# InhwanBae/EigenTrajectory

Hardware: AMD Instinct MI355X
Metric: trajectories/sec fit+project+reconstruct+kmeans (higher is better)
Workload: dtype f32

## Files before the change

### eigentrajectory_amd/csrc/et_fit.hip

```cpp
#include "et_common.h"

namespace et {

constexpr int kFitThreads = 256;

template <int TO, int TP>
struct GramLayout {
    static constexpr int DO = 2 * TO, DP = 2 * TP, D = DO + DP;
    static constexpr int kPairs = 10;
    static constexpr int kSums = kPairs * 64;
    static constexpr int kPartial = kSums + 1;
};
__host__ __device__ constexpr int gram4_block(int s, int q) { return s == 0 ? q : 4 + (s == 1 ? q : (s == 2 ? (q < 2 ? 4 + q : q - 2) : 2 + q)); }
__host__ __device__ constexpr int gram4_pair(int qa, int qb) { return qa * 4 - qa * (qa - 1) / 2 + (qb - qa); }

constexpr int kWaveGramThreads = 256;

__device__ __forceinline__ float4 ld_rows(const float4 *p) { return *p; }

typedef float f32x2_t __attribute__((ext_vector_type(2)));
struct NormPk {
    f32x2_t o, cc, sn, sc;
    __device__ __forceinline__ explicit NormPk(const RowNorm &p)
        : o{p.ox, p.oy}, cc{p.c, p.c}, sn{p.s, -p.s}, sc{p.mv ? p.sca : 1.0f, p.mv ? p.sca : 1.0f} {}
    __device__ __forceinline__ f32x2_t point(f32x2_t xy) const {
        const f32x2_t t = xy - o;
        return (t * cc + __builtin_shufflevector(t, t, 1, 0) * sn) * sc;
    }
    __device__ __forceinline__ float4 quad(float x0, float y0, float x1, float y1) const {
        const f32x2_t a = point((f32x2_t){x0, y0}), b = point((f32x2_t){x1, y1});
        return make_float4(a.x, a.y, b.x, b.y);
    }
};

template <int TO, int TP>
__global__ __launch_bounds__(kWaveGramThreads) void gram_wave_kernel(
    const float *__restrict__ obs, const float *__restrict__ pred, int64_t N, int mode, float static_dist, int which,
    double *__restrict__ partials) {
    using L = GramLayout<TO, TP>;
    static_assert(TO == 8 && TP == 12, "the MFMA tiling below is laid out for 16 + 24 features");
    constexpr int DO = L::DO, DP = L::DP;
    constexpr int QO = DO / 4, QP = DP / 4;
    constexpr int kWaves = kWaveGramThreads / 64;
    constexpr int PR = QO + QP + 1;
    static_assert(PR % 2 == 1, "the row pitch must be odd in float4 units");
    constexpr int kSliceF4 = 64 * PR;
    constexpr int kRedDoubles = kWaves * L::kSums;
    constexpr int kLdsDoubles = (2 * kWaves * kSliceF4 > kRedDoubles ? 2 * kWaves * kSliceF4 : kRedDoubles) + 2;
    __shared__ __attribute__((aligned(16))) double sMem[kLdsDoubles];
    double *sRed = sMem;
    int *sCountPtr = reinterpret_cast<int *>(sMem + kLdsDoubles - 2);

    const int tid = threadIdx.x;
    const int lane = tid & 63, wave = tid >> 6;
    const int kslot = lane >> 4;
    float4 *sRow = reinterpret_cast<float4 *>(sMem) + wave * kSliceF4;
    double acc[L::kPairs];
#pragma unroll
    for (int t = 0; t < L::kPairs; ++t) acc[t] = 0.0;
    const int opi = lane & 3, opslot = (lane >> 2) & 3;
    const int rowA = kslot == 0 ? 0 : (kslot == 1 ? 3 : (kslot == 2 ? 6 : 1)), rowB = rowA ^ 4;
    int offA[4], offB[4];
#pragma unroll
    for (int q = 0; q < 4; ++q) {
        offA[q] = rowA * (4 * PR) + 4 * gram4_block(opslot, q) + opi;
        offB[q] = rowB * (4 * PR) + 4 * gram4_block(opslot, q) + opi;
    }
    int my_count = 0;
    const int64_t n_tiles = ceil_div(N, (int64_t)64);
    const int64_t first = (int64_t)blockIdx.x * kWaves + wave, stride = (int64_t)gridDim.x * kWaves;
    float4 ro[QO], rp[QP];
    auto fetch = [&](int64_t tile) {
        const int64_t n0 = tile * 64;
        const int rows = (int)min((int64_t)64, N - n0);
        const float4 *go = reinterpret_cast<const float4 *>(obs + n0 * DO);
        const float4 *gp = reinterpret_cast<const float4 *>(pred + n0 * DP);
        if (rows == 64) {
#pragma unroll
            for (int j = 0; j < QO; ++j) ro[j] = ld_rows(go + lane + j * 64);
#pragma unroll
            for (int j = 0; j < QP; ++j) rp[j] = ld_rows(gp + lane + j * 64);
        } else {
#pragma unroll
            for (int j = 0; j < QO; ++j) ro[j] = lane + j * 64 < rows * QO ? ld_rows(go + lane + j * 64) : make_float4(0.f, 0.f, 0.f, 0.f);
#pragma unroll
            for (int j = 0; j < QP; ++j) rp[j] = lane + j * 64 < rows * QP ? ld_rows(gp + lane + j * 64) : make_float4(0.f, 0.f, 0.f, 0.f);
        }
    };
    auto wave_sync = [&]() {
        __builtin_amdgcn_fence(__ATOMIC_RELEASE, "wavefront");
        __builtin_amdgcn_wave_barrier();
        __builtin_amdgcn_fence(__ATOMIC_ACQUIRE, "wavefront");
    };
    if (first < n_tiles) fetch(first);
    for (int64_t tile = first; tile < n_tiles; tile += stride) {
        const int rows = (int)min((int64_t)64, N - tile * 64);
        wave_sync();
#pragma unroll
        for (int j = 0; j < QO; ++j) {
            const int q = lane + j * 64;
            sRow[(q / QO) * PR + (q % QO)] = ro[j];
        }
#pragma unroll
        for (int j = 0; j < QP; ++j) {
            const int q = lane + j * 64;
            sRow[(q / QP) * PR + QO + (q % QP)] = rp[j];
        }
        if (tile + stride < n_tiles) fetch(tile + stride);
        wave_sync();
        float4 *orow = sRow + lane * PR, *prow = orow + QO;
        bool use = false;
        if (lane < rows) {
            float xo[DO];
#pragma unroll
            for (int j = 0; j < QO; ++j) {
                const float4 v = orow[j];
                xo[4 * j] = v.x;
                xo[4 * j + 1] = v.y;
                xo[4 * j + 2] = v.z;
                xo[4 * j + 3] = v.w;
            }
            const float ox = xo[DO - 2], oy = xo[DO - 1];
            const RowNorm p = row_norm(ox, oy, ox - xo[DO - 6], oy - xo[DO - 5], mode, static_dist);
            use = p.mv == which;
            if (use) {
                const NormPk np(p);
#pragma unroll
                for (int j = 0; j < QO; ++j) orow[j] = np.quad(xo[4 * j], xo[4 * j + 1], xo[4 * j + 2], xo[4 * j + 3]);
#pragma unroll
                for (int q = 0; q < QP; ++q) {
                    const float4 v = prow[q];
                    prow[q] = np.quad(v.x, v.y, v.z, v.w);
                }
                ++my_count;
            }
        }
        if (!use) {
            const float4 z = make_float4(0.f, 0.f, 0.f, 0.f);
#pragma unroll
            for (int j = 0; j < QO; ++j) orow[j] = z;
#pragma unroll
            for (int q = 0; q < QP; ++q) prow[q] = z;
        }
        wave_sync();
        const float *fb = reinterpret_cast<const float *>(sRow);
#pragma unroll
        for (int g = 0; g < 16; ++g) {
            const int wo = (g >> 1) * (8 * 4 * PR);
            double v[4];
#pragma unroll
            for (int q = 0; q < 4; ++q) v[q] = (double)fb[((g & 1) ? offB[q] : offA[q]) + wo];
#pragma unroll
            for (int qa = 0; qa < 4; ++qa)
#pragma unroll
                for (int qb = qa; qb < 4; ++qb)
                    acc[gram4_pair(qa, qb)] = __builtin_amdgcn_mfma_f64_4x4x4f64(v[qa], v[qb], acc[gram4_pair(qa, qb)], 0, 0, 0);
        }
    }

    __syncthreads();
    if (tid == 0) *sCountPtr = 0;
    __syncthreads();
#pragma unroll
    for (int t = 0; t < L::kPairs; ++t) sRed[wave * L::kSums + t * 64 + lane] = acc[t];
    if (my_count) atomicAdd(sCountPtr, my_count);
    __syncthreads();
    double *dst = partials + (size_t)blockIdx.x * L::kPartial;
    for (int i = tid; i < L::kSums; i += kWaveGramThreads) {
        double sum = 0.0;
        for (int w = 0; w < kWaves; ++w) sum += sRed[w * L::kSums + i];
        dst[i] = sum;
    }
    if (tid == 0) dst[L::kSums] = (double)*sCountPtr;
}

__device__ __forceinline__ double gram4_slot_entry(const double *S, int s, int pa, int ia, int pb, int jb) {
    if (pa > pb || (pa == pb && ia > jb)) {
        int t = pa;
        pa = pb;
        pb = t;
        t = ia;
        ia = jb;
        jb = t;
    }
    return S[gram4_pair(pa, pb) * 64 + jb + 4 * s + 16 * ia];
}
__device__ __forceinline__ double gram_obs_entry(const double *S, int i, int j) { return gram4_slot_entry(S, 0, i >> 2, i & 3, j >> 2, j & 3); }
__device__ __forceinline__ double gram_pred_entry(const double *S, int i, int j) {
    if (i > j) {
        const int t = i;
        i = j;
        j = t;
    }
    const int ba = i >> 2, bb = j >> 2;
    for (int s = 1; s < 4; ++s) {
        int pa = -1, pb = -1;
        for (int q = 0; q < 4; ++q) {
            if (gram4_block(s, q) == 4 + ba) pa = q;
            if (gram4_block(s, q) == 4 + bb) pb = q;
        }
        if (pa >= 0 && pb >= 0) return gram4_slot_entry(S, s, pa, i & 3, pb, j & 3);
    }
    return 0.0;
}

__global__ __launch_bounds__(64) void gram_reduce_kernel(const double *__restrict__ partials, int n_partials, int stride,
                                                         double *__restrict__ sums) {
    const int e = blockIdx.x;
    double s = 0.0;
    for (int b = threadIdx.x; b < n_partials; b += 64) s += partials[(size_t)b * stride + e];
    for (int o = 32; o > 0; o >>= 1) s += __shfl_xor(s, o);
    if (threadIdx.x == 0) sums[e] = s;
}

template <int TO, int TP>
__global__ __launch_bounds__(kFitThreads) void gram_finish_kernel(const double *__restrict__ sSum,
                                                                  double *__restrict__ G_obs,
                                                                  double *__restrict__ G_pred,
                                                                  int64_t *__restrict__ count) {
    using L = GramLayout<TO, TP>;
    constexpr int DO = L::DO, DP = L::DP;
    for (int e = threadIdx.x; e < DO * DO; e += kFitThreads) G_obs[e] = gram_obs_entry(sSum, e / DO, e % DO);
    for (int e = threadIdx.x; e < DP * DP; e += kFitThreads) G_pred[e] = gram_pred_entry(sSum, e / DP, e % DP);
    if (threadIdx.x == 0) *count = (int64_t)sSum[L::kSums];
}

__global__ __launch_bounds__(kFitThreads) void gram_generic_kernel(
    const float *__restrict__ obs, const float *__restrict__ pred, int64_t N, int T_obs, int T_pred, int mode,
    float static_dist, int which, double *__restrict__ partials) {
    constexpr int kSlab = 32;
    const int DO = 2 * T_obs, DP = 2 * T_pred, D = DO + DP;
    extern __shared__ __attribute__((aligned(16))) double sF[];
    int &sCnt = *reinterpret_cast<int *>(sF + kSlab * D);
    const int tid = threadIdx.x;
    const int n_entries = DO * DO + DP * DP;
    double *dst = partials + (size_t)blockIdx.x * (n_entries + 1);
    for (int e = tid; e < n_entries + 1; e += kFitThreads) dst[e] = 0.0;
    if (tid == 0) sCnt = 0;
    const int64_t n_slabs = ceil_div(N, (int64_t)kSlab);
    for (int64_t slab = blockIdx.x; slab < n_slabs; slab += gridDim.x) {
        const int64_t n0 = slab * kSlab;
        const int rows = (int)min((int64_t)kSlab, N - n0);
        __syncthreads();
        if (tid < kSlab) {
            double *f = sF + tid * D;
            bool use = false;
            if (tid < rows) {
                const float *row = obs + (n0 + tid) * DO;
                const float ox = row[DO - 2], oy = row[DO - 1];
                const RowNorm p = row_norm(ox, oy, ox - row[DO - 6], oy - row[DO - 5], mode, static_dist);
                use = p.mv == which;
                if (use) {
                    for (int t = 0; t < T_obs; ++t) {
                        float a, b;
                        normalize_point(p, row[2 * t], row[2 * t + 1], a, b);
                        f[2 * t] = (double)a;
                        f[2 * t + 1] = (double)b;
                    }
                    const float *prow = pred + (n0 + tid) * DP;
                    for (int t = 0; t < T_pred; ++t) {
                        float a, b;
                        normalize_point(p, prow[2 * t], prow[2 * t + 1], a, b);
                        f[DO + 2 * t] = (double)a;
                        f[DO + 2 * t + 1] = (double)b;
                    }
                    atomicAdd(&sCnt, 1);
                }
            }
            if (!use)
                for (int e = 0; e < D; ++e) f[e] = 0.0;
        }
        __syncthreads();
        for (int e = tid; e < n_entries; e += kFitThreads) {
            int i, j;
            if (e < DO * DO) {
                i = e / DO;
                j = e % DO;
            } else {
                const int r = e - DO * DO;
                i = DO + r / DP;
                j = DO + r % DP;
            }
            double s = dst[e];
            for (int r = 0; r < kSlab; ++r) s = fma(sF[r * D + i], sF[r * D + j], s);
            dst[e] = s;
        }
    }
    __syncthreads();
    if (tid == 0) dst[n_entries] = (double)sCnt;
}

__global__ __launch_bounds__(kFitThreads) void gram_generic_finish_kernel(const double *__restrict__ sums, int DO, int DP,
                                                                          double *__restrict__ G_obs,
                                                                          double *__restrict__ G_pred,
                                                                          int64_t *__restrict__ count) {
    const int n_entries = DO * DO + DP * DP;
    for (int e = threadIdx.x; e < n_entries + 1; e += kFitThreads) {
        const double s = sums[e];
        if (e < DO * DO) G_obs[e] = s;
        else if (e < n_entries) G_pred[e - DO * DO] = s;
        else *count = (int64_t)s;
    }
}

constexpr int kJacobiMaxSweeps = 30;
constexpr double kJacobiStop = 1e-10;
constexpr int kEighThreads = 1024;

__device__ __forceinline__ void sqrt_rsqrt(double x, double &root, double &rroot) {
    const double y = __builtin_amdgcn_rsq(x);
    double g = x * y, h = 0.5 * y;
    double r = fma(-h, g, 0.5);
    g = fma(g, r, g);
    h = fma(h, r, h);
    r = fma(-h, g, 0.5);
    g = fma(g, r, g);
    h = fma(h, r, h);
    root = g;
    rroot = h + h;
}

__device__ __forceinline__ void jacobi_schedule(int m, int r, int i, int &p, int &q) {
    int a, b;
    if (i == 0) {
        a = m - 1;
        b = r;
    } else {
        a = r + i;
        a = a >= m - 1 ? a - (m - 1) : a;
        b = r + (m - 1) - i;
        b = b >= m - 1 ? b - (m - 1) : b;
    }
    p = a < b ? a : b;
    q = a < b ? b : a;
}

struct JacobiPair {
    int a, b;
    bool fixed;
    __device__ __forceinline__ void init(int m, int i) {
        fixed = i == 0;
        a = i;
        b = i == 0 ? 0 : m - 1 - i;
    }
    __device__ __forceinline__ void get(int m, int &p, int &q) const {
        const int ae = fixed ? m - 1 : a;
        p = ae < b ? ae : b;
        q = ae < b ? b : ae;
    }
    __device__ __forceinline__ void step(int m) {
        const unsigned a1 = (unsigned)a + 1u, b1 = (unsigned)b + 1u, w = (unsigned)(m - 1);
        a = (int)min(a1, a1 - w);
        b = (int)min(b1, b1 - w);
    }
};

template <class GLoad>
__device__ __forceinline__ void eigh_topk_body(GLoad gload, int n, int k, float *__restrict__ U, float *__restrict__ sigma,
                                               double *sm) {
    const int lane = threadIdx.x;
    const int m = (n + 1) & ~1, half = m / 2;
    double *Abuf = sm;
    double *V = sm + 2 * m * m;
    double *sC = V + m * m;
    double *sS = sC + 64;
    unsigned long long *sMax = reinterpret_cast<unsigned long long *>(sS + 64);
    int *sAct = reinterpret_cast<int *>(sMax + 4);
    int *sUsed = sAct + 64;
    uint2 *sTab = reinterpret_cast<uint2 *>(sUsed + 64);
    for (int i = lane; i < m * m; i += kEighThreads) {
        const int r = i / m, c = i - r * m;
        Abuf[i] = (r < n && c < n) ? gload(r, c) : 0.0;
        V[i] = (r == c && r < n) ? 1.0 : 0.0;
    }
    if (lane < 4) sMax[lane] = 0ull;
    const int nItems = 3 * half;
    for (int idx = lane; idx < (m - 1) * nItems; idx += kEighThreads) {
        const int r = idx / nItems, it = idx - r * nItems, e = it / half, Lt = it - e * half;
        int p, q;
        jacobi_schedule(m, r + 1 == m - 1 ? 0 : r + 1, Lt, p, q);
        int i1 = 0, p1 = 0, q1 = 0, i2 = 0, p2 = 0, q2 = 0;
        for (int i = 0; i < half; ++i) {
            int pi, qi;
            jacobi_schedule(m, r, i, pi, qi);
            if (p == pi || p == qi) { i1 = i; p1 = pi; q1 = qi; }
            if (q == pi || q == qi) { i2 = i; p2 = pi; q2 = qi; }
        }
        const int iR = e == 2 ? i2 : i1, pR = e == 2 ? p2 : p1, qR = e == 2 ? q2 : q1;
        const int iC = e == 1 ? i1 : i2, pC = e == 1 ? p1 : p2, qC = e == 1 ? q1 : q2;
        const unsigned row2 = (e == 2 ? q : p) == qR, col2 = (e == 1 ? p : q) == qC, zero = e == 0 && i1 == i2;
        sTab[idx] = make_uint2((unsigned)(pR * m + pC) | (unsigned)(pR * m + qC) << 12 | (unsigned)iR << 24,
                               (unsigned)(qR * m + pC) | (unsigned)(qR * m + qC) << 12 | (unsigned)iC << 24 | row2 << 29 |
                                   col2 << 30 | zero << 31);
    }
    __syncthreads();
    static_assert(kEighThreads == 1024, "the V items are dealt to wavefronts 4 ... 14 of sixteen");
    constexpr int kVPerSlot = 9 * 64;
    constexpr int kSlots = (32 * 64 + kVPerSlot - 1) / kVPerSlot;
    constexpr int kBlkSlots = (32 * 32 + kEighThreads - 1) / kEighThreads;
    constexpr int kChkSlots = (64 * 64 + kEighThreads - 1) / kEighThreads;
    constexpr int kParBase = kEighThreads - 64;
    int slot_i[kSlots], slot_row[kSlots], blk_1[kBlkSlots], blk_2[kBlkSlots], chk[kChkSlots];
#pragma unroll
    for (int t = 0; t < kSlots; ++t) {
        const int w = lane >> 6;
        const int e = (w >= 4 && (w & 3) != 3) ? ((w - 4) - ((w - 4) >> 2)) * 64 + (lane & 63) + t * kVPerSlot : -1;
        const bool ok = e >= 0 && e < half * n;
        slot_i[t] = ok ? e / n : -1;
        slot_row[t] = ok ? (e % n) * m : 0;
    }
#pragma unroll
    for (int t = 0; t < kBlkSlots; ++t) {
        const int b = lane + t * kEighThreads;
        blk_1[t] = b < half * half ? b / half : -1;
        blk_2[t] = b < half * half ? b % half : 0;
    }
    JacobiPair b1[kBlkSlots], b2[kBlkSlots];
#pragma unroll
    for (int t = 0; t < kBlkSlots; ++t) {
        b1[t].init(m, blk_1[t] < 0 ? 0 : blk_1[t]);
        b2[t].init(m, blk_2[t]);
    }
    const int pl = lane - kParBase;
    const bool split = 4 * half <= 64;
    const bool is_par = pl >= 0 && (split ? (pl & 3) == 0 && (pl >> 2) < half : pl < half);
    const int L = is_par ? (split ? pl >> 2 : pl) : 0;
    const int item0 = pl < 0 ? 0 : (split ? ((pl & 3) < 3 && (pl >> 2) < half ? (pl & 3) * half + (pl >> 2) : 0) : (pl < half ? pl : 0));
    JacobiPair par;
    par.init(m, L);
#pragma unroll
    for (int t = 0; t < kChkSlots; ++t) {
        const int e = lane + t * kEighThreads;
        const int i = e / n, j = e - i * n;
        chk[t] = (e < n * n && j >= i) ? (i * m + j) | (i == j ? 1 << 20 : 0) : -1;
    }
    auto rotation = [&](double apq, double app, double aqq, int buf) {
        const double alpha = aqq - app, beta = 2.0 * apq;
        double h, rh;
        sqrt_rsqrt(alpha * alpha + beta * beta, h, rh);
        const double D = fabs(alpha) + h;
        double g, rg;
        sqrt_rsqrt(D * D + beta * beta, g, rg);
        const double sgn = (alpha == 0.0 || ((alpha > 0.0) == (beta > 0.0))) ? 1.0 : -1.0;
        const bool act = apq != 0.0;
        sC[buf * 32 + L] = act ? D * rg : 1.0;
        sS[buf * 32 + L] = act ? sgn * fabs(beta) * rg : 0.0;
        sAct[buf * 32 + L] = act ? 1 : 0;
    };
    int cur = 0, pb = 0;
    if (pl >= 0) __builtin_amdgcn_s_setprio(3);
    if (is_par) {
        int p, q;
        par.get(m, p, q);
        rotation(Abuf[__mul24(p, m) + q], Abuf[__mul24(p, m) + p], Abuf[__mul24(q, m) + q], 0);
    }
    uint2 ent[3] = {sTab[item0], sTab[split ? item0 : half + item0], sTab[split ? item0 : 2 * half + item0]};
    for (int sweep = 0; sweep < kJacobiMaxSweeps; ++sweep) {
        const double *Ac = Abuf + cur * m * m;
        unsigned long long *mx = sMax + 2 * (sweep & 1);
#pragma unroll
        for (int t = 0; t < kChkSlots; ++t) {
            if (chk[t] < 0) continue;
            const unsigned long long bits = static_cast<unsigned long long>(__double_as_longlong(fabs(Ac[chk[t] & 0xfffff])));
            atomicMax(mx + (chk[t] >> 20), bits);
        }
        if (lane < 2) sMax[2 * ((sweep + 1) & 1) + lane] = 0ull;
        __syncthreads();
        const double off = __longlong_as_double(static_cast<long long>(mx[0])), diag = __longlong_as_double(static_cast<long long>(mx[1]));
        if (off <= kJacobiStop * diag) break;
        for (int r = 0; r < m - 1; ++r) {
            const double *Ar = Abuf + cur * m * m;
            double *Aw = Abuf + (cur ^ 1) * m * m;
            const double *pC = sC + pb * 32, *pS = sS + pb * 32;
            const int *pAct = sAct + pb * 32;
            if (pl >= 0) {
                auto entry = [&](uint2 t) -> double {
                    const double x_pp = Ar[t.x & 0xfffu], x_pq = Ar[(t.x >> 12) & 0xfffu];
                    const double x_qp = Ar[t.y & 0xfffu], x_qq = Ar[(t.y >> 12) & 0xfffu];
                    const int iR = (int)((t.x >> 24) & 31u), iC = (int)((t.y >> 24) & 31u);
                    const double cR = pC[iR], sR = pS[iR], cC = pC[iC], sC_ = pS[iC];
                    const int actR = pAct[iR];
                    const bool row2 = (t.y >> 29) & 1u, col2 = (t.y >> 30) & 1u;
                    const double alR = row2 ? sR : cR, beR = row2 ? cR : -sR;
                    const double alC = col2 ? sC_ : cC, beC = col2 ? cC : -sC_;
                    const double v = alC * (alR * x_pp + beR * x_qp) + beC * (alR * x_pq + beR * x_qq);
                    return ((t.y >> 31) & (unsigned)actR) ? 0.0 : v;
                };
                double apq, app, aqq;
                if (split) {
                    const double v = entry(ent[0]);
                    const int lo = __double2loint(v), hi = __double2hiint(v);
                    apq = v;
                    app = __hiloint2double(__builtin_amdgcn_mov_dpp(hi, 0x55, 0xf, 0xf, false), __builtin_amdgcn_mov_dpp(lo, 0x55, 0xf, 0xf, false));
                    aqq = __hiloint2double(__builtin_amdgcn_mov_dpp(hi, 0xaa, 0xf, 0xf, false), __builtin_amdgcn_mov_dpp(lo, 0xaa, 0xf, 0xf, false));
                } else {
                    apq = entry(ent[0]);
                    app = entry(ent[1]);
                    aqq = entry(ent[2]);
                }
                const int rn = r + 1 == m - 1 ? 0 : r + 1;
                ent[0] = sTab[rn * nItems + item0];
                if (!split) {
                    ent[1] = sTab[rn * nItems + half + item0];
                    ent[2] = sTab[rn * nItems + 2 * half + item0];
                }
                if (is_par) rotation(apq, app, aqq, pb ^ 1);
            }
#pragma unroll
            for (int t = 0; t < kBlkSlots; ++t) {
                const int i1 = blk_1[t], i2 = blk_2[t];
                if (i1 < 0) continue;
                int p1, q1, p2, q2;
                b1[t].get(m, p1, q1);
                b2[t].get(m, p2, q2);
                const int rp = __mul24(p1, m), rq = __mul24(q1, m);
                const int diag_act = pAct[i1] & (i1 == i2 ? 1 : 0);
                const double c1 = pC[i1], s1 = pS[i1], c2 = pC[i2], s2 = pS[i2];
                const double x_pp = Ar[rp + p2], x_pq = Ar[rp + q2], x_qp = Ar[rq + p2], x_qq = Ar[rq + q2];
                const double t_pp = c1 * x_pp - s1 * x_qp, t_qp = s1 * x_pp + c1 * x_qp;
                const double t_pq = c1 * x_pq - s1 * x_qq, t_qq = s1 * x_pq + c1 * x_qq;
                const double r_pp = c2 * t_pp - s2 * t_pq, r_qp = c2 * t_qp - s2 * t_qq;
                double r_pq = s2 * t_pp + c2 * t_pq, r_qp2 = r_qp;
                const double r_qq = s2 * t_qp + c2 * t_qq;
                if (diag_act) {
                    r_pq = 0.0;
                    r_qp2 = 0.0;
                }
                Aw[rp + p2] = r_pp;
                Aw[rp + q2] = r_pq;
                Aw[rq + p2] = r_qp2;
                Aw[rq + q2] = r_qq;
            }
#pragma unroll
            for (int t = 0; t < kSlots; ++t) {
                const int i = slot_i[t];
                if (i < 0) continue;
                int p, q;
                jacobi_schedule(m, r, i, p, q);
                const double c = pC[i], sn = pS[i];
                double *row = V + slot_row[t];
                const double vjp = row[p], vjq = row[q];
                row[p] = c * vjp - sn * vjq;
                row[q] = sn * vjp + c * vjq;
            }
#pragma unroll
            for (int t = 0; t < kBlkSlots; ++t) {
                b1[t].step(m);
                b2[t].step(m);
            }
            __syncthreads();
            cur ^= 1;
            pb ^= 1;
        }
    }
    double *A = Abuf + cur * m * m;
    __syncthreads();
    if (lane < n) {
        const double di = A[lane * m + lane];
        int rank = 0;
        for (int i = 0; i < n; ++i) {
            const double dj = A[i * m + i];
            rank += (dj > di || (dj == di && i < lane)) ? 1 : 0;
        }
        sUsed[lane] = rank;
    }
    __syncthreads();
    for (int e = lane; e < n * k; e += kEighThreads) {
        const int col = e / k, j = e - col * k;
        if (sUsed[col] != j) continue;
        int im = 0;
        for (int i = 1; i < n; ++i)
            if (fabs(V[i * m + col]) > fabs(V[im * m + col])) im = i;
        const double sgn = V[im * m + col] < 0.0 ? -1.0 : 1.0;
        const double lam = A[col * m + col];
        sigma[j] = (float)sqrt(lam > 0.0 ? lam : 0.0);
        for (int i = 0; i < n; ++i) U[i * k + j] = (float)(sgn * V[i * m + col]);
    }
}

__global__ __launch_bounds__(kEighThreads) void eigh_topk_kernel(const double *__restrict__ G, int n, int k,
                                                                  float *__restrict__ U, float *__restrict__ sigma) {
    extern __shared__ __attribute__((aligned(16))) double eigh_smem[];
    eigh_topk_body([=](int r, int c) { return G[r * n + c]; }, n, k, U, sigma, eigh_smem);
}

struct EighBatch {
    const double *G[ET_EIGH_MAX_BATCH];
    float *U[ET_EIGH_MAX_BATCH];
    float *sigma[ET_EIGH_MAX_BATCH];
    int n[ET_EIGH_MAX_BATCH];
    int k[ET_EIGH_MAX_BATCH];
};

__global__ __launch_bounds__(kEighThreads) void eigh_topk_batch_kernel(const EighBatch b) {
    extern __shared__ __attribute__((aligned(16))) double eigh_smem[];
    const int i = blockIdx.x;
    const double *G = b.G[i];
    const int n = b.n[i];
    eigh_topk_body([=](int r, int c) { return G[r * n + c]; }, n, b.k[i], b.U[i], b.sigma[i], eigh_smem);
}

template <int TO, int TP>
__global__ __launch_bounds__(kEighThreads) void fit_finish_eigh_kernel(const double *__restrict__ sums, int k,
                                                                       double *__restrict__ G_obs, double *__restrict__ G_pred,
                                                                       int64_t *__restrict__ count, float *__restrict__ U_obs,
                                                                       float *__restrict__ U_pred, float *__restrict__ sigma_obs,
                                                                       float *__restrict__ sigma_pred) {
    using L = GramLayout<TO, TP>;
    constexpr int DO = L::DO, DP = L::DP;
    extern __shared__ __attribute__((aligned(16))) double eigh_smem[];
    double *sT = eigh_smem;
    const bool is_pred = blockIdx.x == 1;
    for (int e = threadIdx.x; e < L::kSums; e += kEighThreads) sT[e] = sums[e];
    if (!is_pred && count && threadIdx.x == 0) *count = (int64_t)sums[L::kSums];
    __syncthreads();
    if (!is_pred) {
        if (G_obs)
            for (int e = threadIdx.x; e < DO * DO; e += kEighThreads) G_obs[e] = gram_obs_entry(sT, e / DO, e % DO);
        eigh_topk_body([=](int r, int c) { return gram_obs_entry(sT, r, c); }, DO, k, U_obs, sigma_obs, eigh_smem + 768);
    } else {
        if (G_pred)
            for (int e = threadIdx.x; e < DP * DP; e += kEighThreads) G_pred[e] = gram_pred_entry(sT, e / DP, e % DP);
        eigh_topk_body([=](int r, int c) { return gram_pred_entry(sT, r, c); }, DP, k, U_pred, sigma_pred, eigh_smem + 768);
    }
}

static int fit_grid(int64_t N) {
    const int64_t tiles = ceil_div(N, (int64_t)kWaveGramThreads);
    return (int)(tiles < 768 ? (tiles > 0 ? tiles : 1) : 768);
}

}

using namespace et;

extern "C" size_t et_fit_gram_workspace_bytes(int64_t N, int T_obs, int T_pred) {
    const size_t DO = 2 * (size_t)T_obs, DP = 2 * (size_t)T_pred;
    const size_t per = DO * DO + DP * DP + 1;
    return sizeof(double) * per * ((size_t)fit_grid(N) + 1);
}

extern "C" size_t et_fit_descriptor_workspace_bytes(int64_t N, int T_obs, int T_pred) {
    const size_t DO = 2 * (size_t)T_obs, DP = 2 * (size_t)T_pred;
    return et_fit_gram_workspace_bytes(N, T_obs, T_pred) + sizeof(double) * (DO * DO + DP * DP + 2);
}

extern "C" int et_fit_gram(const float *obs, const float *pred, int64_t N, int T_obs, int T_pred, int mode,
                           float static_dist, int which, double *G_obs, double *G_pred, int64_t *count,
                           void *workspace, size_t workspace_bytes, et_stream_t stream) {
    if (N < 0 || T_obs < 3 || T_obs > ET_MAX_T || T_pred < 1 || T_pred > ET_MAX_T || mode < 0 || mode > 3 ||
        (which != 0 && which != 1) || !G_obs || !G_pred || !count)
        return ET_ERR_INVALID_ARG;
    if (N > 0 && (!obs || !pred)) return ET_ERR_INVALID_ARG;
    if (workspace_bytes < et_fit_gram_workspace_bytes(N, T_obs, T_pred) || !workspace) return ET_ERR_WORKSPACE;
    hipStream_t st = (hipStream_t)stream;
    const int DO = 2 * T_obs, DP = 2 * T_pred;
    if (N == 0) {
        ET_HIP_TRY(hipMemsetAsync(G_obs, 0, sizeof(double) * DO * DO, st));
        ET_HIP_TRY(hipMemsetAsync(G_pred, 0, sizeof(double) * DP * DP, st));
        ET_HIP_TRY(hipMemsetAsync(count, 0, sizeof(int64_t), st));
        return ET_OK;
    }
    const int grid = fit_grid(N);
    double *partials = (double *)workspace;
    if (T_obs == 8 && T_pred == 12 && aligned16(obs) && aligned16(pred)) {
        hipLaunchKernelGGL((gram_wave_kernel<8, 12>), dim3(grid), dim3(kWaveGramThreads), 0, st, obs, pred, N, mode,
                           static_dist, which, partials);
        ET_LAUNCH_CHECK();
        constexpr int per = GramLayout<8, 12>::kPartial;
        double *sums = partials + (size_t)grid * per;
        hipLaunchKernelGGL(gram_reduce_kernel, dim3(per), dim3(64), 0, st, partials, grid, per, sums);
        ET_LAUNCH_CHECK();
        hipLaunchKernelGGL((gram_finish_kernel<8, 12>), dim3(1), dim3(kFitThreads), 0, st, sums, G_obs, G_pred, count);
    } else {
        const size_t lds = sizeof(double) * (32 * (size_t)(DO + DP) + 1);
        hipLaunchKernelGGL(gram_generic_kernel, dim3(grid), dim3(kFitThreads), lds, st, obs, pred, N, T_obs, T_pred,
                           mode, static_dist, which, partials);
        ET_LAUNCH_CHECK();
        const int per = DO * DO + DP * DP + 1;
        double *sums = partials + (size_t)grid * per;
        hipLaunchKernelGGL(gram_reduce_kernel, dim3(per), dim3(64), 0, st, partials, grid, per, sums);
        ET_LAUNCH_CHECK();
        hipLaunchKernelGGL(gram_generic_finish_kernel, dim3(1), dim3(kFitThreads), 0, st, sums, DO, DP, G_obs, G_pred,
                           count);
    }
    ET_LAUNCH_CHECK();
    return ET_OK;
}

static size_t eigh_lds_bytes(int n) {
    const size_t m = ((size_t)n + 1) & ~(size_t)1;
    return sizeof(double) * (3 * m * m + 128 + 4) + sizeof(int) * (64 + 64) + sizeof(uint2) * (m - 1) * 3 * (m / 2);
}

extern "C" int et_eigh_topk_batch(int batch, const double *const *G, const int *n, const int *k, float *const *U,
                                  float *const *sigma, et_stream_t stream) {
    if (batch < 0 || batch > ET_EIGH_MAX_BATCH || (batch > 0 && (!G || !n || !k || !U || !sigma))) return ET_ERR_INVALID_ARG;
    if (batch == 0) return ET_OK;
    EighBatch b;
    size_t lds = 0;
    for (int i = 0; i < batch; ++i) {
        if (!G[i] || !U[i] || !sigma[i] || n[i] < 1 || n[i] > 64 || k[i] < 1 || k[i] > n[i]) return ET_ERR_INVALID_ARG;
        b.G[i] = G[i];
        b.U[i] = U[i];
        b.sigma[i] = sigma[i];
        b.n[i] = n[i];
        b.k[i] = k[i];
        const size_t need = eigh_lds_bytes(n[i]);
        lds = need > lds ? need : lds;
    }
    if (lds > 48 * 1024)
        ET_HIP_TRY(hipFuncSetAttribute(reinterpret_cast<const void *>(eigh_topk_batch_kernel),
                                       hipFuncAttributeMaxDynamicSharedMemorySize, (int)lds));
    hipLaunchKernelGGL(eigh_topk_batch_kernel, dim3(batch), dim3(kEighThreads), lds, (hipStream_t)stream, b);
    ET_LAUNCH_CHECK();
    return ET_OK;
}

extern "C" int et_eigh_topk(const double *G, int n, int k, float *U, float *sigma, et_stream_t stream) {
    if (!G || !U || !sigma || n < 1 || n > 64 || k < 1 || k > n) return ET_ERR_INVALID_ARG;
    const size_t lds = eigh_lds_bytes(n);
    if (lds > 48 * 1024)
        ET_HIP_TRY(hipFuncSetAttribute(reinterpret_cast<const void *>(eigh_topk_kernel),
                                       hipFuncAttributeMaxDynamicSharedMemorySize, (int)lds));
    hipLaunchKernelGGL(eigh_topk_kernel, dim3(1), dim3(kEighThreads), lds, (hipStream_t)stream, G, n, k, U, sigma);
    ET_LAUNCH_CHECK();
    return ET_OK;
}

extern "C" int et_fit_descriptor(const float *obs, const float *pred, int64_t N, int T_obs, int T_pred, int k, int mode,
                                 float static_dist, int which, float *U_obs, float *U_pred, float *sigma_obs,
                                 float *sigma_pred, double *G_obs, double *G_pred, int64_t *count, void *workspace,
                                 size_t workspace_bytes, et_stream_t stream) {
    if (!U_obs || !U_pred || !sigma_obs || !sigma_pred || k < 1 || T_obs < 3 || T_obs > ET_MAX_T || T_pred < 1 || T_pred > ET_MAX_T ||
        k > 2 * T_obs || k > 2 * T_pred)
        return ET_ERR_INVALID_ARG;
    hipStream_t st = (hipStream_t)stream;
    const bool fused = N > 0 && T_obs == 8 && T_pred == 12 && obs && pred && aligned16(obs) && aligned16(pred) && mode >= 0 &&
                       mode <= 3 && (which == 0 || which == 1);
    if (!fused) {
        const size_t gram_ws = et_fit_gram_workspace_bytes(N, T_obs, T_pred);
        const size_t DO = 2 * (size_t)T_obs, DP = 2 * (size_t)T_pred;
        if (!workspace || workspace_bytes < et_fit_descriptor_workspace_bytes(N, T_obs, T_pred)) return ET_ERR_WORKSPACE;
        double *tail = reinterpret_cast<double *>(static_cast<char *>(workspace) + gram_ws);
        double *go = G_obs ? G_obs : tail, *gp = G_pred ? G_pred : tail + DO * DO;
        int64_t *cn = count ? count : reinterpret_cast<int64_t *>(tail + DO * DO + DP * DP);
        const int rc = et_fit_gram(obs, pred, N, T_obs, T_pred, mode, static_dist, which, go, gp, cn, workspace, gram_ws, stream);
        if (rc) return rc;
        const double *Gs[2] = {go, gp};
        const int ns[2] = {(int)DO, (int)DP}, ks[2] = {k, k};
        float *Us[2] = {U_obs, U_pred}, *ss[2] = {sigma_obs, sigma_pred};
        return et_eigh_topk_batch(2, Gs, ns, ks, Us, ss, stream);
    }
    if (!workspace || workspace_bytes < et_fit_descriptor_workspace_bytes(N, T_obs, T_pred)) return ET_ERR_WORKSPACE;
    const int grid = fit_grid(N);
    double *partials = (double *)workspace;
    hipLaunchKernelGGL((gram_wave_kernel<8, 12>), dim3(grid), dim3(kWaveGramThreads), 0, st, obs, pred, N, mode, static_dist, which,
                       partials);
    ET_LAUNCH_CHECK();
    constexpr int per = GramLayout<8, 12>::kPartial;
    double *sums = partials + (size_t)grid * per;
    hipLaunchKernelGGL(gram_reduce_kernel, dim3(per), dim3(64), 0, st, partials, grid, per, sums);
    ET_LAUNCH_CHECK();
    const size_t lds = sizeof(double) * 768 + eigh_lds_bytes(24);
    if (lds > 48 * 1024)
        ET_HIP_TRY(hipFuncSetAttribute(reinterpret_cast<const void *>(fit_finish_eigh_kernel<8, 12>),
                                       hipFuncAttributeMaxDynamicSharedMemorySize, (int)lds));
    hipLaunchKernelGGL((fit_finish_eigh_kernel<8, 12>), dim3(2), dim3(kEighThreads), lds, st, sums, k, G_obs, G_pred, count, U_obs,
                       U_pred, sigma_obs, sigma_pred);
    ET_LAUNCH_CHECK();
    return ET_OK;
}
```

Measured before the change: 2.038 billion.

## Restructure MFMA Gram tiling to skip cross blocks and prestage fp64 planes

Reworks the f64 MFMA Gram kernel so that each tile is processed in two 32-row halves. Normalized rows are written into LDS already converted to double and laid out in planes. The block-pair assignment is changed to 6 operands per slot and 8 pair accumulators, so obs×pred cross products are no longer computed and every needed block pair is computed exactly once, which a static_assert checks. LDS reads go through inline asm ds_read_b64 with manual waitcnt pipelining, which overlaps loads with MFMAs. This adds inline-asm fragility, and the tail fetch now uses clamped loads.

```diff
diff --git a/eigentrajectory_amd/csrc/et_fit.hip b/eigentrajectory_amd/csrc/et_fit.hip
--- a/eigentrajectory_amd/csrc/et_fit.hip
+++ b/eigentrajectory_amd/csrc/et_fit.hip
@@ -7,18 +7,27 @@
 template <int TO, int TP>
 struct GramLayout {
     static constexpr int DO = 2 * TO, DP = 2 * TP, D = DO + DP;
-    static constexpr int kPairs = 10;
+    static constexpr int kPairs = 8;
     static constexpr int kSums = kPairs * 64;
     static constexpr int kPartial = kSums + 1;
 };
-__host__ __device__ constexpr int gram4_block(int s, int q) { return s == 0 ? q : 4 + (s == 1 ? q : (s == 2 ? (q < 2 ? 4 + q : q - 2) : 2 + q)); }
-__host__ __device__ constexpr int gram4_pair(int qa, int qb) { return qa * 4 - qa * (qa - 1) / 2 + (qb - qa); }
+__host__ __device__ constexpr int gram4_block(int s, int q) {
+    if (q >= 4) return s == 0 ? q - 2 : (s == 1 ? 2 : (s == 2 ? 3 : 6));
+    return s == 0 ? q : 4 + (s == 1 ? q : (s == 2 ? (q < 2 ? 4 + q : q - 2) : 2 + q));
+}
+__host__ __device__ constexpr int gram4_qa(int t) { return t == 7 ? 4 : (t < 2 ? 0 : (t < 3 ? 1 : (t < 5 ? 0 : 1))); }
+__host__ __device__ constexpr int gram4_qb(int t) { return t == 7 ? 5 : (t == 0 ? 0 : (t < 3 ? 1 : (t == 3 || t == 5 ? 2 : 3))); }
+__host__ __device__ constexpr int gram4_plane(int block) {
+    constexpr int idx[10] = {0, 1, 4, 5, 9, 8, 2, 6, 3, 7};
+    return idx[block];
+}
 
 constexpr int kWaveGramThreads = 256;
 
 __device__ __forceinline__ float4 ld_rows(const float4 *p) { return *p; }
 
 typedef float f32x2_t __attribute__((ext_vector_type(2)));
+typedef double f64x2_t __attribute__((ext_vector_type(2)));
 struct NormPk {
     f32x2_t o, cc, sn, sc;
     __device__ __forceinline__ explicit NormPk(const RowNorm &p)
@@ -32,6 +41,13 @@
         return make_float4(a.x, a.y, b.x, b.y);
     }
 };
+
+template <int IMM>
+__device__ __forceinline__ double lds_read_f64(int addr) {
+    double d;
+    asm volatile("ds_read_b64 %0, %1 offset:%2" : "=v"(d) : "v"(addr), "n"(IMM) : "memory");
+    return d;
+}
 
 template <int TO, int TP>
 __global__ __launch_bounds__(kWaveGramThreads) void gram_wave_kernel(
@@ -44,47 +60,66 @@
     constexpr int kWaves = kWaveGramThreads / 64;
     constexpr int PR = QO + QP + 1;
     static_assert(PR % 2 == 1, "the row pitch must be odd in float4 units");
-    constexpr int kSliceF4 = 64 * PR;
+    constexpr int kHalf = 32;
+    constexpr int kPlaneBytes = (kHalf + 2) * 16;
+    constexpr int kSliceBytes = 2 * (QO + QP) * kPlaneBytes;
+    static_assert(kHalf * PR * 16 <= kSliceBytes, "the fp32 stage-in rows live inside the slice");
     constexpr int kRedDoubles = kWaves * L::kSums;
-    constexpr int kLdsDoubles = (2 * kWaves * kSliceF4 > kRedDoubles ? 2 * kWaves * kSliceF4 : kRedDoubles) + 2;
+    constexpr int kLdsDoubles = (kWaves * kSliceBytes / 8 > kRedDoubles ? kWaves * kSliceBytes / 8 : kRedDoubles) + 2;
     __shared__ __attribute__((aligned(16))) double sMem[kLdsDoubles];
     double *sRed = sMem;
     int *sCountPtr = reinterpret_cast<int *>(sMem + kLdsDoubles - 2);
 
     const int tid = threadIdx.x;
-    const int lane = tid & 63, wave = tid >> 6;
+    const int lane = tid & 63, wave = __builtin_amdgcn_readfirstlane(tid >> 6);
     const int kslot = lane >> 4;
-    float4 *sRow = reinterpret_cast<float4 *>(sMem) + wave * kSliceF4;
+    char *sSlice = reinterpret_cast<char *>(sMem) + wave * kSliceBytes;
+    float4 *sRow = reinterpret_cast<float4 *>(sSlice);
     double acc[L::kPairs];
 #pragma unroll
     for (int t = 0; t < L::kPairs; ++t) acc[t] = 0.0;
     const int opi = lane & 3, opslot = (lane >> 2) & 3;
     const int rowA = kslot == 0 ? 0 : (kslot == 1 ? 3 : (kslot == 2 ? 6 : 1)), rowB = rowA ^ 4;
-    int offA[4], offB[4];
-#pragma unroll
-    for (int q = 0; q < 4; ++q) {
-        offA[q] = rowA * (4 * PR) + 4 * gram4_block(opslot, q) + opi;
-        offB[q] = rowB * (4 * PR) + 4 * gram4_block(opslot, q) + opi;
-    }
+    const int sliceAddr = (int)(uintptr_t)(__attribute__((address_space(3))) char *)sSlice;
+    int offA[6], offB[6];
+#pragma unroll
+    for (int q = 0; q < 6; ++q) {
+        const int plane = 2 * gram4_plane(gram4_block(opslot, q)) + (opi >> 1);
+        offA[q] = sliceAddr + plane * kPlaneBytes + rowA * 16 + (opi & 1) * 8;
+        offB[q] = sliceAddr + plane * kPlaneBytes + rowB * 16 + (opi & 1) * 8;
+    }
+    const int crow = lane & (kHalf - 1), chh = lane >> 5;
+    int offW[5];
+#pragma unroll
+    for (int j = 0; j < 5; ++j) offW[j] = 2 * gram4_plane(chh * 5 + j) * kPlaneBytes + crow * 16;
     int my_count = 0;
     const int64_t n_tiles = ceil_div(N, (int64_t)64);
     const int64_t first = (int64_t)blockIdx.x * kWaves + wave, stride = (int64_t)gridDim.x * kWaves;
-    float4 ro[QO], rp[QP];
-    auto fetch = [&](int64_t tile) {
-        const int64_t n0 = tile * 64;
-        const int rows = (int)min((int64_t)64, N - n0);
+    constexpr int FO = QO / 2, FP = QP / 2;
+    auto fetch = [&](int64_t tile, int half, float4 (&ro)[FO], float4 (&rp)[FP]) {
+        const int64_t n0 = tile * 64 + half * kHalf;
+        const int rows = (int)max((int64_t)0, min((int64_t)kHalf, N - n0));
         const float4 *go = reinterpret_cast<const float4 *>(obs + n0 * DO);
         const float4 *gp = reinterpret_cast<const float4 *>(pred + n0 * DP);
-        if (rows == 64) {
-#pragma unroll
-            for (int j = 0; j < QO; ++j) ro[j] = ld_rows(go + lane + j * 64);
-#pragma unroll
-            for (int j = 0; j < QP; ++j) rp[j] = ld_rows(gp + lane + j * 64);
+        if (rows == kHalf) {
+#pragma unroll
+            for (int j = 0; j < FO; ++j) ro[j] = ld_rows(go + lane + j * 64);
+#pragma unroll
+            for (int j = 0; j < FP; ++j) rp[j] = ld_rows(gp + lane + j * 64);
         } else {
-#pragma unroll
-            for (int j = 0; j < QO; ++j) ro[j] = lane + j * 64 < rows * QO ? ld_rows(go + lane + j * 64) : make_float4(0.f, 0.f, 0.f, 0.f);
-#pragma unroll
-            for (int j = 0; j < QP; ++j) rp[j] = lane + j * 64 < rows * QP ? ld_rows(gp + lane + j * 64) : make_float4(0.f, 0.f, 0.f, 0.f);
+            const float4 *bo = rows > 0 ? go : reinterpret_cast<const float4 *>(obs);
+            const float4 *bp = rows > 0 ? gp : reinterpret_cast<const float4 *>(pred);
+            const int lo = rows > 0 ? rows * QO - 1 : 0, lp = rows > 0 ? rows * QP - 1 : 0;
+            auto clamped = [](int i, int last) {
+                int c = min(i, last);
+                asm volatile("" : "+v"(c));
+                return c;
+            };
+#pragma unroll
+            for (int j = 0; j < FO; ++j) ro[j] = ld_rows(bo + clamped(lane + j * 64, lo));
+#pragma unroll
+            for (int j = 0; j < FP; ++j) rp[j] = ld_rows(bp + clamped(lane + j * 64, lp));
+            asm volatile("");
         }
     };
     auto wave_sync = [&]() {
@@ -92,69 +127,86 @@
         __builtin_amdgcn_wave_barrier();
         __builtin_amdgcn_fence(__ATOMIC_ACQUIRE, "wavefront");
     };
-    if (first < n_tiles) fetch(first);
+    float4 ro2[2][FO], rp2[2][FP];
+    if (first < n_tiles) {
+        fetch(first, 0, ro2[0], rp2[0]);
+        fetch(first, 1, ro2[1], rp2[1]);
+    }
     for (int64_t tile = first; tile < n_tiles; tile += stride) {
-        const int rows = (int)min((int64_t)64, N - tile * 64);
-        wave_sync();
-#pragma unroll
-        for (int j = 0; j < QO; ++j) {
-            const int q = lane + j * 64;
-            sRow[(q / QO) * PR + (q % QO)] = ro[j];
-        }
-#pragma unroll
-        for (int j = 0; j < QP; ++j) {
-            const int q = lane + j * 64;
-            sRow[(q / QP) * PR + QO + (q % QP)] = rp[j];
-        }
-        if (tile + stride < n_tiles) fetch(tile + stride);
-        wave_sync();
-        float4 *orow = sRow + lane * PR, *prow = orow + QO;
-        bool use = false;
-        if (lane < rows) {
-            float xo[DO];
-#pragma unroll
-            for (int j = 0; j < QO; ++j) {
-                const float4 v = orow[j];
-                xo[4 * j] = v.x;
-                xo[4 * j + 1] = v.y;
-                xo[4 * j + 2] = v.z;
-                xo[4 * j + 3] = v.w;
-            }
-            const float ox = xo[DO - 2], oy = xo[DO - 1];
-            const RowNorm p = row_norm(ox, oy, ox - xo[DO - 6], oy - xo[DO - 5], mode, static_dist);
-            use = p.mv == which;
-            if (use) {
-                const NormPk np(p);
-#pragma unroll
-                for (int j = 0; j < QO; ++j) orow[j] = np.quad(xo[4 * j], xo[4 * j + 1], xo[4 * j + 2], xo[4 * j + 3]);
-#pragma unroll
-                for (int q = 0; q < QP; ++q) {
-                    const float4 v = prow[q];
-                    prow[q] = np.quad(v.x, v.y, v.z, v.w);
+#pragma unroll
+        for (int half = 0; half < 2; ++half) {
+            float4(&ro)[FO] = ro2[half], (&rp)[FP] = rp2[half];
+            const int rows = (int)max((int64_t)0, min((int64_t)kHalf, N - tile * 64 - half * kHalf));
+            wave_sync();
+#pragma unroll
+            for (int j = 0; j < FO; ++j) {
+                const int q = lane + j * 64;
+                sRow[(q / QO) * PR + (q % QO)] = ro[j];
+            }
+#pragma unroll
+            for (int j = 0; j < FP; ++j) {
+                const int q = lane + j * 64;
+                sRow[(q / QP) * PR + QO + (q % QP)] = rp[j];
+            }
+            fetch(tile + stride, half, ro, rp);
+            wave_sync();
+            float4 x[5];
+            {
+                const float4 *row = sRow + crow * PR;
+                const float4 o2 = row[QO - 2], o3 = row[QO - 1];
+#pragma unroll
+                for (int j = 0; j < 5; ++j) x[j] = row[chh * 5 + j];
+                bool use = false;
+                if (crow < rows) {
+                    const float ox = o3.z, oy = o3.w;
+                    const RowNorm p = row_norm(ox, oy, ox - o2.z, oy - o2.w, mode, static_dist);
+                    use = p.mv == which;
+                    if (use) {
+                        const NormPk np(p);
+#pragma unroll
+                        for (int j = 0; j < 5; ++j) x[j] = np.quad(x[j].x, x[j].y, x[j].z, x[j].w);
+                        my_count += 1 - chh;
+                    }
                 }
-                ++my_count;
-            }
-        }
-        if (!use) {
-            const float4 z = make_float4(0.f, 0.f, 0.f, 0.f);
-#pragma unroll
-            for (int j = 0; j < QO; ++j) orow[j] = z;
-#pragma unroll
-            for (int q = 0; q < QP; ++q) prow[q] = z;
-        }
-        wave_sync();
-        const float *fb = reinterpret_cast<const float *>(sRow);
-#pragma unroll
-        for (int g = 0; g < 16; ++g) {
-            const int wo = (g >> 1) * (8 * 4 * PR);
-            double v[4];
-#pragma unroll
-            for (int q = 0; q < 4; ++q) v[q] = (double)fb[((g & 1) ? offB[q] : offA[q]) + wo];
-#pragma unroll
-            for (int qa = 0; qa < 4; ++qa)
-#pragma unroll
-                for (int qb = qa; qb < 4; ++qb)
-                    acc[gram4_pair(qa, qb)] = __builtin_amdgcn_mfma_f64_4x4x4f64(v[qa], v[qb], acc[gram4_pair(qa, qb)], 0, 0, 0);
+                if (!use) {
+#pragma unroll
+                    for (int j = 0; j < 5; ++j) x[j] = make_float4(0.f, 0.f, 0.f, 0.f);
+                }
+            }
+            wave_sync();
+#pragma unroll
+            for (int j = 0; j < 5; ++j) {
+                *reinterpret_cast<f64x2_t *>(sSlice + offW[j]) = (f64x2_t){(double)x[j].x, (double)x[j].y};
+                *reinterpret_cast<f64x2_t *>(sSlice + offW[j] + kPlaneBytes) = (f64x2_t){(double)x[j].z, (double)x[j].w};
+            }
+            wave_sync();
+            double v[2][6];
+            auto issue = [&](auto G) {
+                constexpr int g = decltype(G)::value;
+#pragma unroll
+                for (int q = 0; q < 6; ++q) v[g & 1][q] = lds_read_f64<(g >> 1) * (8 * 16)>((g & 1) ? offB[q] : offA[q]);
+            };
+            auto group = [&](auto G) {
+                constexpr int g = decltype(G)::value;
+                if constexpr (g < 7) issue(std::integral_constant<int, g + 1>{});
+                double *u = v[g & 1];
+                if constexpr (g < 7)
+                    asm volatile("s_waitcnt lgkmcnt(6)" : "+v"(u[0]), "+v"(u[1]), "+v"(u[2]), "+v"(u[3]), "+v"(u[4]), "+v"(u[5]));
+                else
+                    asm volatile("s_waitcnt lgkmcnt(0)" : "+v"(u[0]), "+v"(u[1]), "+v"(u[2]), "+v"(u[3]), "+v"(u[4]), "+v"(u[5]));
+#pragma unroll
+                for (int t = 0; t < L::kPairs; ++t)
+                    acc[t] = __builtin_amdgcn_mfma_f64_4x4x4f64(u[gram4_qa(t)], u[gram4_qb(t)], acc[t], 0, 0, 0);
+            };
+            issue(std::integral_constant<int, 0>{});
+            group(std::integral_constant<int, 0>{});
+            group(std::integral_constant<int, 1>{});
+            group(std::integral_constant<int, 2>{});
+            group(std::integral_constant<int, 3>{});
+            group(std::integral_constant<int, 4>{});
+            group(std::integral_constant<int, 5>{});
+            group(std::integral_constant<int, 6>{});
+            group(std::integral_constant<int, 7>{});
         }
     }
 
@@ -174,35 +226,55 @@
     if (tid == 0) dst[L::kSums] = (double)*sCountPtr;
 }
 
-__device__ __forceinline__ double gram4_slot_entry(const double *S, int s, int pa, int ia, int pb, int jb) {
-    if (pa > pb || (pa == pb && ia > jb)) {
-        int t = pa;
-        pa = pb;
-        pb = t;
-        t = ia;
+struct GramPairTable {
+    short where[10][10];
+};
+constexpr GramPairTable gram4_make_pairs() {
+    GramPairTable tab{};
+    for (int ba = 0; ba < 10; ++ba)
+        for (int bb = 0; bb < 10; ++bb) {
+            tab.where[ba][bb] = -1;
+            for (int s = 0; s < 4; ++s)
+                for (int t = 0; t < (s == 3 ? 7 : 8); ++t) {
+                    const int A = gram4_block(s, gram4_qa(t)), B = gram4_block(s, gram4_qb(t));
+                    if (A == ba && B == bb)
+                        tab.where[ba][bb] = (short)(64 * t + 4 * s);
+                    else if (A == bb && B == ba)
+                        tab.where[ba][bb] = (short)(64 * t + 4 * s + 1024);
+                }
+        }
+    return tab;
+}
+__device__ constexpr GramPairTable kGramPairs = gram4_make_pairs();
+__device__ __forceinline__ double gram4_entry(const double *S, int ba, int ia, int bb, int jb) {
+    if (ba == bb && ia > jb) {
+        const int t = ia;
         ia = jb;
         jb = t;
     }
-    return S[gram4_pair(pa, pb) * 64 + jb + 4 * s + 16 * ia];
-}
-__device__ __forceinline__ double gram_obs_entry(const double *S, int i, int j) { return gram4_slot_entry(S, 0, i >> 2, i & 3, j >> 2, j & 3); }
+    const int w = kGramPairs.where[ba][bb];
+    return (w & 1024) ? S[(w & 1023) + ia + 16 * jb] : S[w + jb + 16 * ia];
+}
+__device__ __forceinline__ double gram_obs_entry(const double *S, int i, int j) { return gram4_entry(S, i >> 2, i & 3, j >> 2, j & 3); }
 __device__ __forceinline__ double gram_pred_entry(const double *S, int i, int j) {
-    if (i > j) {
-        const int t = i;
-        i = j;
-        j = t;
-    }
-    const int ba = i >> 2, bb = j >> 2;
-    for (int s = 1; s < 4; ++s) {
-        int pa = -1, pb = -1;
-        for (int q = 0; q < 4; ++q) {
-            if (gram4_block(s, q) == 4 + ba) pa = q;
-            if (gram4_block(s, q) == 4 + bb) pb = q;
-        }
-        if (pa >= 0 && pb >= 0) return gram4_slot_entry(S, s, pa, i & 3, pb, j & 3);
-    }
-    return 0.0;
-}
+    return gram4_entry(S, 4 + (i >> 2), i & 3, 4 + (j >> 2), j & 3);
+}
+__host__ __device__ constexpr int gram4_times_computed(int ba, int bb) {
+    int n = 0;
+    for (int s = 0; s < 4; ++s)
+        for (int t = 0; t < (s == 3 ? 7 : 8); ++t) {
+            const int A = gram4_block(s, gram4_qa(t)), B = gram4_block(s, gram4_qb(t));
+            n += (A == ba && B == bb) || (A == bb && B == ba);
+        }
+    return n;
+}
+__host__ __device__ constexpr bool gram4_covers_once() {
+    for (int ba = 0; ba < 10; ++ba)
+        for (int bb = ba; bb < 10; ++bb)
+            if (gram4_times_computed(ba, bb) != ((ba < 4) == (bb < 4) ? 1 : 0)) return false;
+    return true;
+}
+static_assert(gram4_covers_once(), "10 + 21 block pairs, each computed once, no observation x prediction product");
 
 __global__ __launch_bounds__(64) void gram_reduce_kernel(const double *__restrict__ partials, int n_partials, int stride,
                                                          double *__restrict__ sums) {
```

Result: no change. 2.026 billion (-0.6%).
